# peterrum/dealii-multigrid

Hardware: AMD Instinct MI355X
Metric: DoF/s per V-cycle, 3D octant p=4 (higher is better)
Workload: dtype f64; 1 GPU; 3D octant (GeometryType quadrant) HMG-global p=4 FP64, NRefGlobal=8, SmootherDegree=3, coarse solver direct, f=1, zero Dirichlet (BASELINE.json configs[2]); n_dofs=137199985, n_cells=2127189, n_levels=9, parallelism=1 GPU, chebyshev_start_vector=deal.II's (i mod 11) - mean on the local numbering, fused_transfer_bricks=33509

## Files before the change

### dealii_multigrid_amd/csrc/kernels_apply.hpp

```cpp
#pragma once
#include "kernels_common.hpp"

namespace mgamd
{
#ifdef MGAMD_KERNEL_DEBUG
#define MGAMD_STAMP(k)                         \
  if (args.stamps && tid == 0)                 \
    args.stamps[(size_t)block * 8 + (k)] = wall_clock64();
#define MGAMD_ABLATED(bit) (args.ablate & (bit))
#else
#define MGAMD_STAMP(k)
#define MGAMD_ABLATED(bit) false
#endif

  template <typename T, int P>
  __device__ __forceinline__ void
  interior_diag_terms(const Mats<P, T> &mats, const int t, T &s_K, T &s_M)
  {
    const int tt[3] = {t % P, (t / P) % P, t / (P * P)};
    T         m[3], k[3];
#pragma unroll
    for (int d = 0; d < 3; ++d)
      {
        T dm = T(0), dk = T(0);
        if (tt[d] == 0)
          {
            dm = T(mats.M[P * (P + 1) + P]) + T(mats.M[0]);
            dk = T(mats.K[P * (P + 1) + P]) + T(mats.K[0]);
          }
#pragma unroll
        for (int q = 1; q < P; ++q)
          if (q == tt[d])
            {
              dm = T(mats.M[q * (P + 1) + q]);
              dk = T(mats.K[q * (P + 1) + q]);
            }
        m[d] = dm;
        k[d] = dk;
      }
    s_K = k[0] * m[1] * m[2] + m[0] * k[1] * m[2] + m[0] * m[1] * k[2];
    s_M = m[0] * m[1] * m[2];
  }

  template <typename T, int P, int B, int MODE, bool CONSTR = false, bool WAVE = false, int NTHREADS = 0, bool MASS = true>
// ... 252 lines not shown
        MGAMD_STAMP(4)
      }
#endif
  }

  template <typename T, int P, int B, int MODE_, bool CONSTR, bool MASS>
  __device__ __forceinline__ void
  lattice_apply_persistent_body(const ApplyArgs<T, P> &args, const uint32_t w, const uint32_t stride, unsigned char *smem_raw)
  {
    using G  = Geo<P, B>;
    using IM = InteriorMap<P, B>;
    static_assert(G::SPW == 1 && G::N_INT > 0, "persistent workgroups: one slot per workgroup");
    constexpr int  MODE   = base_mode(MODE_);
    constexpr bool FUSE_R = MODE_ == MODE_RESIDUAL_RESTRICT, FUSE_P = MODE_ == MODE_CHEB_PROLONGATE, FUSE = FUSE_R || FUSE_P;
    static_assert(!FUSE || (!CONSTR && B >= 2 && G::ABLOCK == 256), "fused transfers: plain bricks, 256 threads");
    static_assert(!CONSTR || P == 1, "constrained bricks larger than a family: p = 1 only (LevelTables::build)");
    static_assert(MODE_ != MODE_MASS || !MASS, "the mass pass has no mass TERM: one instantiation, MASS = false");
    constexpr int BC = B >= 2 ? B / 2 : 1, NC = P * BC + 1, NC3 = NC * NC * NC;
    T *bufA = reinterpret_cast<T *>(smem_raw);
    T *bufB = bufA + G::N3;
    T *dtab = bufB + G::N3;

    constexpr int BLOCK = G::ABLOCK;
    constexpr int ITER  = (G::N_INT + BLOCK - 1) / BLOCK;
    constexpr int ITERS = (G::N_SHELL + BLOCK - 1) / BLOCK;
    constexpr int ITC   = FUSE ? (NC3 + BLOCK - 1) / BLOCK : 1;
    constexpr int P3    = P * P * P;
    static_assert(!FUSE || 2 * ITERS <= 15, "two flag bits per shell entry in a 16-bit word");

    const int      tid = threadIdx.x;
    const uint32_t n   = args.g.n_slots;
    if (w >= n)
      return;

    if (is_cheb(MODE))
      {
        for (int t = tid; t < P3; t += BLOCK)
          {
            T sv, s_M;
            interior_diag_terms<T, P>(args.m, t, sv, s_M);
            dtab[t]      = sv;
            dtab[P3 + t] = T(1) / sv;
          }
      }
    constexpr int NI = IM::NI_;
    struct InteriorWalk
    {
      int x, y, z;
      __device__ __forceinline__ int
      pos() const
      {
        return (z * G::N + y) * G::N + x;
      }
      __device__ __forceinline__ int
      type() const
      {
        return (x % P) + P * ((y % P) + P * (z % P));
      }
      __device__ __forceinline__ void
      next()
      {
        constexpr int DZ = BLOCK / (NI * NI), DY = (BLOCK % (NI * NI)) / NI, DX = BLOCK % NI;
        x += DX;
        if (x > NI)
          {
            x -= NI;
            ++y;
          }
        y += DY;
        if (y > NI)
          {
            y -= NI;
            ++z;
          }
        z += DZ;
      }
    };
    const InteriorWalk walk0{tid % NI + 1, (tid / NI) % NI + 1, tid / (NI * NI) + 1};
    auto has_entry = [&](int it) -> bool { return (it + 1) * BLOCK <= G::N_INT || tid + it * BLOCK < G::N_INT; };
    int spos[ITERS];
#pragma unroll
    for (int it = 0; it < ITERS; ++it)
      {
        const int idx = tid + it * BLOCK;
        spos[it]      = idx < G::N_SHELL ? (int)args.g.shell_pos[idx] : -1;
      }
    __syncthreads();

    constexpr bool x_from_b = MODE == MODE_CHEB_FIRST;
    auto load_tables = [&](uint32_t v, uint32_t &slot, uint32_t &base, uint32_t(&sg)[ITERS], double &h, uint32_t &fm, uint32_t &fl,
                           uint32_t(&cg)[ITC]) {
      slot = xcd_contiguous(v, n);
      base = args.g.interior_base[slot];
      h    = args.g.h[slot];
      fm   = 0;
      fl   = 0;
      if constexpr (FUSE)
        {
          fl = args.fused.flags[(size_t)slot * BLOCK + tid];
          const uint32_t *__restrict__ c0 = args.fused.coarse_idx + (size_t)slot * NC3;
#pragma unroll
          for (int it = 0; it < ITC; ++it)
            cg[it] = NT_LOAD(c0 + min(tid + it * BLOCK, NC3 - 1));
        }
      if constexpr (brick_may_be_constrained(B, CONSTR))
        if (args.g.fmask != nullptr)
          fm = args.g.fmask[slot];
      const uint32_t *__restrict__ p0 = args.g.shell_idx + (size_t)slot * G::N_SHELL;
#pragma unroll
      for (int it = 0; it < ITERS; ++it)
        {
          if ((it + 1) * BLOCK <= G::N_SHELL)
            sg[it] = NT_LOAD(p0 + it * BLOCK + tid);
          else
            sg[it] = NT_LOAD(p0 + min(tid + it * BLOCK, G::N_SHELL - 1));
        }
    };
    auto load_values = [&](uint32_t base, const uint32_t(&sg)[ITERS], const uint32_t fl, const uint32_t(&cg)[ITC], T(&xv)[ITER], T(&sv)[ITERS],
                           T(&sbv)[ITERS], T(&cv)[ITC]) {
      const T *__restrict__ in = x_from_b ? args.epi.b : args.src;
#pragma unroll
      for (int it = 0; it < ITER; ++it)
        xv[it] = NT_LOAD(&in[base + (uint32_t)(has_entry(it) ? tid + it * BLOCK : 0)]);
#pragma unroll
      for (int it = 0; it < ITERS; ++it)
        {
          const uint32_t gi = sg[it] < args.gather_limit ? sg[it] : 0;
          sv[it]            = in[gi];
          if (x_from_b)
            sbv[it] = args.epi.dinv[gi];
          if (FUSE_R)
            sbv[it] = args.epi.b[((fl >> (2 * it)) & 1u) ? gi : 0];
        }
      if constexpr (FUSE_P)
        {
#pragma unroll
          for (int it = 0; it < ITC; ++it)
            cv[it] = args.fused.coarse[cg[it] != DEV_INVALID ? cg[it] : 0];
        }
    };

    uint32_t slot, base, sgi[ITERS], fmcur, flcur, cgi[ITC];
    double   hcur;
    T        xg[ITER], sval[ITERS], sb[ITERS], cval[ITC];
    load_tables(w, slot, base, sgi, hcur, fmcur, flcur, cgi);
    load_values(base, sgi, flcur, cgi, xg, sval, sb, cval);

    for (uint32_t v = w;;)
      {
        const uint32_t block    = v;
        (void)block;
        const uint32_t vn       = v + stride;
        const bool     has_next = vn < n;
        MGAMD_STAMP(0)
        const T rh = T(1) / T(hcur);
        if constexpr (MASS && is_cheb(MODE))
          {
            const T c = T(args.sigma) * T(args.g.q[slot]);
            for (int t = tid; t < P3; t += BLOCK)
              {
                T s_K, s_M;
                interior_diag_terms<T, P>(args.m, t, s_K, s_M);
                const T sv   = s_K + c * s_M;
                dtab[t]      = sv;
                dtab[P3 + t] = T(1) / sv;
              }
            if (x_from_b)
              __syncthreads();
          }
        auto interior_dinv = [&](int t) -> T {
          return fabs((double)dtab[t]) > 1.0e-10 * fabs((double)rh) ? rh * dtab[P3 + t] : T(1);
        };
        const bool fused_slot = FUSE && ((__builtin_amdgcn_readfirstlane((int)flcur) >> 15) & 1);
        T          bv[ITER], xo[ITER];
        uint32_t slotn = slot, basen = base, sgn[ITERS], fmn = fmcur, fln = flcur, cgn[ITC];
        double   hn = hcur;
        if (has_next)
          load_tables(vn, slotn, basen, sgn, hn, fmn, fln, cgn);
        {
#pragma unroll
          for (int it = 0; it < ITER; ++it)
            {
              const uint32_t g = base + (uint32_t)(has_entry(it) ? tid + it * BLOCK : 0);
              xo[it]           = T(0);
              bv[it]           = x_from_b ? xg[it] : T(0);
              if (MODE == MODE_CHEB && !FUSE_P && args.epi.xold)
                xo[it] = NT_LOAD(&args.epi.xold[g]);
// ... 53 lines not shown
                    const uint32_t f2 = (flcur >> (2 * it)) & 3u;
                    if (!(f2 & 2u))
                      sval[it] += bufB[spos[it]];
                    if (f2 & 1u)
                      args.fused.scratch[sgi[it]] = sval[it];
                  }
              InteriorWalk wk = walk0;
#pragma unroll
              for (int it = 0; it < ITER; ++it, wk.next())
                if (has_entry(it))
                  {
                    xg[it] += bufB[wk.pos()];
                    NT_STORE(xg[it], &args.fused.x_inout[base + (uint32_t)(tid + it * BLOCK)]);
                  }
            }
        if (x_from_b)
          {
#pragma unroll
            for (int it = 0; it < ITERS; ++it)
              sval[it] = args.epi.c0 * sb[it] * sval[it];
          }
#pragma unroll
        for (int it = 0; it < ITERS; ++it)
          if (spos[it] >= 0)
            bufA[spos[it]] = sgi[it] < args.gather_limit ? sval[it] : T(0);
        {
          InteriorWalk wk = walk0;
#pragma unroll
          for (int it = 0; it < ITER; ++it, wk.next())
            if (has_entry(it))
              bufA[wk.pos()] = x_from_b ? args.epi.c0 * interior_dinv(wk.type()) * bv[it] : xg[it];
        }
        __syncthreads();
        MGAMD_STAMP(1)

        bool any_hanging = false;
        if constexpr (brick_may_be_constrained(B, CONSTR))
          {
            any_hanging = fmcur != 0;
            if (any_hanging)
              brick_constraint_passes<T, P, B, BLOCK>(bufA, args.m, tid, 1, args.g.fmask + slot, false, &fmcur);
          }
        if constexpr (MODE == MODE_MASS)
          mass_sweeps<T, P, B, BLOCK, true, true, false>(bufA, args.m, tid, 1, &hcur, false);
        else
          lattice_sweeps<T, P, B, BLOCK, NoHook, true, (MODE != MODE_CHEB || sizeof(T) == 4), false, MASS>(
            bufA, bufB, args.m, tid, 1, &hcur, NoHook(), false, args.sigma, args.g.q + slot);
        if constexpr (brick_may_be_constrained(B, CONSTR))
          if (any_hanging)
            brick_constraint_passes<T, P, B, BLOCK>(bufA, args.m, tid, 1, args.g.fmask + slot, true, &fmcur);
        MGAMD_STAMP(2)

        T xgn[ITER], svaln[ITERS], sbn[ITERS], cvaln[ITC];
        if (has_next)
          load_values(basen, sgn, fln, cgn, xgn, svaln, sbn, cvaln);

        if (FUSE_R && fused_slot)
          {
            if constexpr (FUSE_R)
              {
                InteriorWalk wk = walk0;
#pragma unroll
                for (int it = 0; it < ITER; ++it, wk.next())
                  if (has_entry(it))
                    bufA[wk.pos()] = bv[it] - bufA[wk.pos()];
#pragma unroll
// ... 52 lines not shown
              if (has_entry(it))
                {
                  const uint32_t g  = base + (uint32_t)(tid + it * BLOCK);
                  const T        ax = bufA[wk.pos()];
                  T              r;
                  if (MODE == MODE_VMULT || MODE == MODE_MASS)
                    r = ax;
                  else if (MODE == MODE_RESIDUAL)
                    r = bv[it] - ax;
                  else
                    {
                      const T dv  = interior_dinv(wk.type());
                      const T xov = MODE == MODE_CHEB_SECOND ? args.epi.c0 * dv * bv[it] : xo[it];
                      const T xv  = x_from_b ? args.epi.c0 * dv * bv[it] : xg[it];
                      if (FUSE_P)
                        r = xv + args.epi.f2 * dv * (bv[it] - ax);
                      else
                        r = xv + args.epi.f1 * (xv - xov) + args.epi.f2 * dv * (bv[it] - ax);
                    }
                  if (MODE == MODE_CHEB && !FUSE_P)
                    store_result(args.epi, g, r);
                  else
                    NT_STORE(r, &args.epi.out[g]);
                }
            MGAMD_STAMP(3)
#pragma unroll
            for (int it = 0; it < ITERS; ++it)
              if (spos[it] >= 0 && sgi[it] < args.scatter_limit)
                atomic_add(&args.tail_acc[sgi[it] - args.n_interior], bufA[spos[it]]);
          }
        MGAMD_STAMP(4)
        if (!has_next)
          break;
        v    = vn;
        slot  = slotn;
        base  = basen;
        hcur  = hn;
        fmcur = fmn;
        flcur = fln;
#pragma unroll
        for (int it = 0; it < ITC; ++it)
          {
            cgi[it]  = cgn[it];
            cval[it] = cvaln[it];
          }
#pragma unroll
        for (int it = 0; it < ITERS; ++it)
          {
            sgi[it]  = sgn[it];
            sval[it] = svaln[it];
            sb[it]   = sbn[it];
          }
#pragma unroll
        for (int it = 0; it < ITER; ++it)
          xg[it] = xgn[it];
        __syncthreads();
      }
  }
#undef MGAMD_STAMP
#undef MGAMD_ABLATED

  constexpr int CELL_WAVES = 4;
  template <typename T, int P>
  constexpr size_t
  cell_wave_lds()
  {
    using G = Geo<P, 1, 64>;
    static_assert(P >= 2, "wave-scoped cells: P >= 2 (at P = 1 the closed-form D^-1 table of lattice_apply_body is per slot, apply_lds_bytes)");
    return (((2 * (size_t)G::SPW * G::N3 + 2 * P * P * P + G::SPW) * sizeof(T) + 15) / 16) * 16;
  }

  constexpr size_t CU_LDS_BYTES = 160 * 1024;
  constexpr int
  wgs_lds_admits(size_t lds_bytes)
  {
    return (int)(CU_LDS_BYTES / lds_bytes);
  }
  constexpr int
  min_of(int a, int b, int c)
  {
    return a < b ? (a < c ? a : c) : (b < c ? b : c);
  }
  template <typename T, int P>
  constexpr size_t
  small_slots_lds_bytes()
  {
    return apply_lds_bytes<T, P, 2>() > CELL_WAVES * cell_wave_lds<T, P>() ? apply_lds_bytes<T, P, 2>() : CELL_WAVES * cell_wave_lds<T, P>();
  }
  template <typename T, int P>
  constexpr int
  brick2_vgpr_cap()
  {
// ... 76 lines not shown
  struct BrickPairArgs
  {
    ApplyArgs<T, P> a;
    SlotGroupDev    g_constrained;
    uint32_t        n_wg_plain;
  };
  static_assert(sizeof(BrickPairArgs<double, MAX_KERNEL_DEGREE>) <= KERNARG_LIMIT, "BrickPairArgs exceeds the kernel-argument segment");
  template <typename T, int P, int B, int MODE>
  __global__ void
  __launch_bounds__((Geo<P, B>::ABLOCK), 1) lattice_apply_pair_kernel(const BrickPairArgs<T, P> args)
  {
    extern __shared__ __align__(16) unsigned char smem_raw[];
    if (blockIdx.x < args.n_wg_plain)
      lattice_apply_body<T, P, B, MODE, false>(args.a, blockIdx.x, args.n_wg_plain, smem_raw);
    else
      {
        ApplyArgs<T, P> a = args.a;
        a.g               = args.g_constrained;
        a.stamps          = nullptr;
        lattice_apply_body<T, P, B, MODE, true>(a, blockIdx.x - args.n_wg_plain, gridDim.x - args.n_wg_plain, smem_raw);
      }
  }

  template <typename T, int P, int B, int MODE, bool MASS>
  __global__ void
  __launch_bounds__((Geo<P, B>::ABLOCK), 2) lattice_apply_persistent_pair_kernel(const BrickPairArgs<T, P> args)
  {
    extern __shared__ __align__(16) unsigned char smem_raw[];
    if (args.n_wg_plain == 0)
      {
        ApplyArgs<T, P> a = args.a;
        a.g               = args.g_constrained;
        a.stamps          = nullptr;
        lattice_apply_persistent_body<T, P, B, base_mode(MODE), true, MASS>(a, blockIdx.x, gridDim.x, smem_raw);
        __syncthreads();
        lattice_apply_persistent_body<T, P, B, MODE, false, MASS>(args.a, blockIdx.x, gridDim.x, smem_raw);
      }
    else if (blockIdx.x < args.n_wg_plain)
      lattice_apply_persistent_body<T, P, B, MODE, false, MASS>(args.a, blockIdx.x, args.n_wg_plain, smem_raw);
    else
      {
        ApplyArgs<T, P> a = args.a;
        a.g               = args.g_constrained;
        a.stamps          = nullptr;
        lattice_apply_persistent_body<T, P, B, base_mode(MODE), true, MASS>(a, blockIdx.x - args.n_wg_plain, gridDim.x - args.n_wg_plain, smem_raw);
      }
  }

  template <typename T, int P>
  struct SmallSlotsArgs
  {
    ApplyArgs<T, P> a;
    SlotGroupDev    g_cells;
    uint32_t        n_wg_bricks;
  };
  static_assert(sizeof(SmallSlotsArgs<double, MAX_KERNEL_DEGREE>) <= KERNARG_LIMIT, "SmallSlotsArgs exceeds the kernel-argument segment");
  template <typename T, int P, int MODE, bool MASS = true>
  __global__ void
  __launch_bounds__(256, (small_slots_wgs_per_cu<T, P>())) lattice_apply_small_kernel(const SmallSlotsArgs<T, P> args)
  {
    extern __shared__ __align__(16) unsigned char smem_raw[];
    if (blockIdx.x < args.n_wg_bricks)
      lattice_apply_body<T, P, 2, MODE, false, false, 256, MASS>(args.a, blockIdx.x, args.n_wg_bricks, smem_raw);
    else
      {
        ApplyArgs<T, P> a = args.a;
        a.g               = args.g_cells;
        a.stamps          = nullptr;
        cell_waves_body<T, P, MODE, MASS>(a, blockIdx.x - args.n_wg_bricks, gridDim.x - args.n_wg_bricks, smem_raw);
      }
  }

  struct CellClusterDev
  {
    const uint32_t *uniq_ptr;
    const uint32_t *uniq_idx;
    const uint16_t *loc;
// ... 683 lines not shown
```

### dealii_multigrid_amd/csrc/kernels_common.hpp

```cpp
#pragma once
#include <hip/hip_runtime.h>
#include <stdint.h>

namespace mgamd
{
  constexpr uint32_t DEV_INVALID = 0xFFFFFFFFu;

  constexpr size_t KERNARG_LIMIT     = 4096;
  constexpr int    MAX_KERNEL_DEGREE = 7;

#ifndef MGAMD_NO_NT_STREAMS
#define NT_LOAD(p) __builtin_nontemporal_load(p)
#define NT_STORE(v, p) __builtin_nontemporal_store(v, p)
#else
#define NT_LOAD(p) (*(p))
#define NT_STORE(v, p) (*(p) = (v))
#endif

  __device__ __forceinline__ uint32_t
  xcd_contiguous(uint32_t b, uint32_t n)
  {
    const uint32_t k = b & 7u, q = n >> 3, r = n & 7u;
    return k * q + (k < r ? k : r) + (b >> 3);
  }

  template <int P, typename S = double>
  struct Mats
  {
    S M[(P + 1) * (P + 1)];
    S K[(P + 1) * (P + 1)];
    S I0[(P + 1) * (P + 1)];
    S I1[(P + 1) * (P + 1)];
    static constexpr int NH = (P + 2) / 2, NO = (P + 1) / 2;
    S                    Me[NH * NH], Mo[NO * NO], Ke[NH * NH], Ko[NO * NO];
  };

  constexpr bool
  brick_may_be_constrained(int B, bool constr)
  {
    return B == 2 || (constr && B > 2);
  }

  template <int P, int B, int THREADS = 256>
  struct Geo
  {
    static constexpr int N       = P * B + 1;
    static constexpr int N3      = N * N * N;
    static constexpr int NI      = N - 2;
    static constexpr int N_INT   = NI > 0 ? NI * NI * NI : 0;
    static constexpr int N_SHELL = N3 - N_INT;
    static constexpr int LINES   = N * N;
    static constexpr int SPW     = LINES >= THREADS ? 1 : THREADS / LINES;
    static constexpr int BLOCK   = ((SPW * LINES + 63) / 64) * 64;
    static constexpr int ABLOCK  = BLOCK > 256 ? 256 : BLOCK;
    static constexpr int ROUNDS  = (SPW * LINES + ABLOCK - 1) / ABLOCK;
  };

// ... 1042 lines not shown
            {
#pragma unroll
              for (int b = 0; b <= P; ++b)
                out[c * P + (mir ? P - b : b)] += T(Eh[ar * (P + 1) + b]) * v;
            }
        }
  }

  template <typename T, int P>
  struct FusedTransferDev
  {
    const uint32_t *flags      = nullptr;
    const uint32_t *coarse_idx = nullptr;
    T               Eh[(P + 1) * (P + 1)];
    T              *coarse  = nullptr;
    T              *x_inout = nullptr;
    T              *scratch = nullptr;
  };

  template <typename T, int P>
  struct ApplyArgs
  {
    SlotGroupDev g;
    Mats<P, T>   m;
    const T     *src;
    T           *tail_acc;
    uint32_t     n_interior;
    unsigned long long *stamps;
    uint32_t     ablate;
    Epilogue<T>  epi;
    uint32_t gather_limit, scatter_limit;
    FusedTransferDev<T, P> fused;
    double sigma = 0.0;
  };
  static_assert(sizeof(ApplyArgs<double, MAX_KERNEL_DEGREE>) <= KERNARG_LIMIT, "ApplyArgs exceeds the kernel-argument segment");

  template <int P, int B, int THREADS = 256>
  struct InteriorMap
  {
    using G                   = Geo<P, B, THREADS>;
    static constexpr int NI_  = G::NI > 0 ? G::NI : 1;
    static constexpr int NIN_ = G::N_INT > 0 ? G::N_INT : 1;
    static constexpr int ITER = (G::SPW * NIN_ + G::ABLOCK - 1) / G::ABLOCK;
    __device__ static __forceinline__ void
    decode(int idx, int nslots, bool &ok, int &sl, int &i, int &lds)
    {
      ok = idx < nslots * NIN_;
      sl = (G::SPW == 1 || !ok) ? 0 : idx / NIN_;
      i  = G::SPW == 1 ? (ok ? idx : 0) : (ok ? idx % NIN_ : 0);
      const int x = i % NI_, y = (i / NI_) % NI_, z = i / (NI_ * NI_);
      lds = sl * G::N3 + ((z + 1) * G::N + (y + 1)) * G::N + x + 1;
    }
  };

}
```

### dealii_multigrid_amd/csrc/level_operator.hpp

```cpp
#pragma once
#include "runtime.hpp"
#include "kernels.hpp"

#include <cmath>
#include <cstring>
#include <map>
#include <mutex>
#include <type_traits>
#include <unordered_map>

namespace mgamd
{
  inline int
  grid_for(size_t n)
  {
    size_t g = (n + 255) / 256;
    if (g > 2048)
      g = 2048;
    if (g < 1)
      g = 1;
    return (int)g;
  }

  template <typename T>
// ... 9 lines not shown
    hipLaunchKernelGGL(vec_dot_final_kernel<>, 1, 256, 0, ctx->stream, ctx->d_partial, g, ctx->d_result);
    HIP_CHECK(hipMemcpyAsync(ctx->h_result, ctx->d_result, sizeof(double), hipMemcpyDeviceToHost, ctx->stream));
    ctx->sync();
    return ctx->h_result[0];
  }

  inline void
  ensure_dynamic_lds(Ctx *ctx, const void *kern, size_t lds)
  {
    static std::mutex                                      m;
    static std::map<std::pair<int, const void *>, size_t> done;
    std::lock_guard<std::mutex>                            lock(m);
    auto                                                   it = done.find({ctx->device, kern});
    if (it != done.end() && it->second >= lds)
      return;
    HIP_CHECK(hipFuncSetAttribute(kern, hipFuncAttributeMaxDynamicSharedMemorySize, (int)lds));
    done[{ctx->device, kern}] = lds;
  }

  template <typename A>
  inline void
  launch_lds(Ctx *ctx, hipStream_t st, void (*kern)(A), int grid, int block, size_t lds, const A &args)
  {
    ensure_dynamic_lds(ctx, reinterpret_cast<const void *>(kern), lds);
    hipLaunchKernelGGL(kern, grid, block, lds, st, args);
  }

  inline int
  resident_workgroups(const Ctx *ctx, int per_cu = 2)
  {
    return std::max(8, per_cu * ctx->n_cu / 8 * 8);
  }

  template <typename A>
  inline void
  launch_persistent(Ctx *ctx, hipStream_t st, void (*kern)(A), int n_work, int per_cu, int block, size_t lds, const A &args)
  {
    launch_lds(ctx, st, kern, std::min(n_work, resident_workgroups(ctx, per_cu)), block, lds, args);
  }

  template <int... Vs, typename F>
  inline bool
  dispatch_value(int v, F &&f)
  {
    return ((v == Vs && (f(std::integral_constant<int, Vs>()), true)) || ...);
  }
  template <typename F>
  inline bool
  dispatch_degree(int p, F &&f)
  {
    return dispatch_value<1, 2, 3, 4, 5, 6, 7>(p, f);
  }
  template <int P, int... Bs, typename F>
  inline bool
  dispatch_brick_size(int B, F &&f)
  {
    return P * B + 1 <= 17 && dispatch_value<Bs...>(B, [&](auto b) {
             if constexpr (P * b() + 1 <= 17)
               f(b);
           });
  }

  template <typename T, int P, int B, int MODE, bool CONSTR = false>
  inline void
  launch_lattice(Ctx *ctx, hipStream_t st, const ApplyArgs<T, P> &a, bool diag)
  {
    using G = Geo<P, B>;
    if (a.g.n_slots == 0)
      return;
    const int grid = (int)((a.g.n_slots + G::SPW - 1) / G::SPW);
    if (diag)
      launch_lds(ctx, st, lattice_diag_kernel<T, P, B, CONSTR>, grid, G::BLOCK, 3 * (size_t)G::SPW * G::N3 * sizeof(T), a);
    else if constexpr (B == 1 && P >= 2)
      {
        using GW = Geo<P, 1, 64>;
        const uint32_t n_w    = (uint32_t)((a.g.n_slots + GW::SPW - 1) / GW::SPW);
        const uint32_t grid_w = (n_w + CELL_WAVES - 1) / CELL_WAVES;
        constexpr size_t lds  = CELL_WAVES * cell_wave_lds<T, P>();
        static_assert(lds <= 64 * 1024, "above the default dynamic-LDS limit the launch has to go through launch_lds");
        hipLaunchKernelGGL((cell_waves_kernel<T, P, MODE>), grid_w, 64 * CELL_WAVES, lds, st, a);
      }
    else if constexpr (persistent_lattice(G::N))
      {
        void (*kern)(ApplyArgs<T, P>) = lattice_apply_persistent_kernel<T, P, B, MODE, CONSTR, false>;
        if constexpr (MODE != MODE_MASS)
          if (a.sigma != 0.0)
            kern = lattice_apply_persistent_kernel<T, P, B, MODE, CONSTR, true>;
        launch_persistent(ctx, st, kern, grid, persistent_wgs_per_cu<T, P>(), G::ABLOCK, apply_lds_bytes<T, P, B>(), a);
      }
    else
      launch_lds(ctx, st, lattice_apply_kernel<T, P, B, MODE, CONSTR>, grid, G::ABLOCK, apply_lds_bytes<T, P, B>(), a);
    HIP_CHECK(hipGetLastError());
  }

  template <typename T>
  struct GroupDev
  {
    int            B = 1, N = 2;
    bool           constrained = false;
    size_t         n_halo      = 0;
    size_t         n_slots = 0;
    DBuf<uint32_t> interior_base, shell_idx;
    DBuf<uint16_t> mask, shell_pos;
    DBuf<double>   h, q, h_cell;
    DBuf<uint32_t> fmask;
    void
    upload_scales(const SlotGroup &g)
    {
      std::vector<double> ah(g.h.size()), ratio(g.h.size());
      bool                any = false;
      for (size_t s = 0; s < g.h.size(); ++s)
        {
          ah[s]    = g.a[s] * g.h[s];
          ratio[s] = g.h[s] * g.h[s] / g.a[s];
          any |= g.a[s] != 1.0;
        }
      h.upload(ah);
      q.upload(ratio);
      if (any)
        h_cell.upload(g.h);
    }
// ... 71 lines not shown
  template <typename T>
  struct FusedTransferHost
  {
    int                 group = -1;
    const uint32_t     *flags = nullptr;
    const uint32_t     *coarse_idx = nullptr;
    uint32_t            nc3 = 0;
    std::vector<double> E;
    const uint8_t      *tail_flags = nullptr;
    const uint32_t     *tail_chunks   = nullptr;
    uint32_t            n_tail_chunks = 0;
    T *coarse = nullptr, *scratch = nullptr, *x_inout = nullptr;
  };
  constexpr bool
  fused_transfer_supported(int p)
  {
    return persistent_brick(p) != 0;
  }

  template <typename T>
  struct LevelOperator : LevelOperatorBase
  {
    int                                       p = 1;
    std::vector<std::unique_ptr<GroupDev<T>>> groups;
    DBuf<T>                                   tail_acc;
    DBuf<uint8_t>                             dinv_code;
    DBuf<T>                                   dinv_table;
    const T                                  *dinv_coded = nullptr;
    int                                       dominant_B = 0;
    uint32_t                                  ablate = 0;
    DBuf<unsigned long long>                  stamps;
    int                                       stamp_mode = -1;
    bool                                      halo_overlap = true;

    struct HaloDev
    {
      DBuf<uint32_t> pack_idx, sh_tail, sh_ptr;
      DBuf<int32_t>  sh_src, sh_owner_src;
      DBuf<T>        send, recv;
    };
    std::unique_ptr<HaloDev> halo;

    struct RobinDev
    {
      DBuf<uint32_t> idx;
      DBuf<uint8_t>  flags;
      DBuf<double>   scale;
      uint32_t       n_faces = 0;
    };
    std::unique_ptr<RobinDev> robin;

    struct DirichletDev
    {
      DBuf<uint32_t> idx;
      DBuf<uint16_t> mask;
      DBuf<double>   scale;
      uint32_t       n_cells = 0;
    };
    std::unique_ptr<DirichletDev> dirichlet;
    struct HangingDev
    {
      DBuf<uint32_t> ptr, col;
      DBuf<double>   val;
      uint32_t       n_rows = 0;
    };
    std::unique_ptr<HangingDev> hanging;

    enum class LaunchKind
    {
      LATTICE,
      LATTICE_CONSTRAINED,
      BRICK_PAIR,
      BRICKS_AND_CELLS,
      BRICKS_AND_CLUSTERS,
      CLUSTERS,
      ROBIN_FACES
    };
    struct LaunchStep
    {
      LaunchKind   kind;
      GroupDev<T> *g, *partner;
      size_t       begin, end;
    };
    struct LaunchPlan
    {
      std::vector<LaunchStep> ordinary, diagonal;
      std::vector<LaunchStep> halo_slots, interior_slots;
    } plan;

    LevelOperator(Ctx *c, const mgamd_dofs *dofs, std::shared_ptr<Comm> cm)
    {
      ctx    = c;
      type   = (int)sizeof(T);
      tables = dofs->tables;
      tria   = dofs->tria;
      p      = tables->p;
      sigma  = tables->sigma;
      if (tables->ls_level && sigma != 0.0)
        throw std::invalid_argument("level operator: mass coefficient " + std::to_string(sigma) +
                                    " on a local-smoothing level: not implemented (refinement-edge matrices have no mass term)");
      if (cm && dofs->halo)
        {
          comm      = cm;
          halo_plan = dofs->halo;
          halo      = std::make_unique<HaloDev>();
          halo->pack_idx.upload(halo_plan->pack_idx);
          halo->sh_tail.upload(halo_plan->sh_tail);
          halo->sh_ptr.upload(halo_plan->sh_ptr);
          halo->sh_src.upload(halo_plan->sh_src);
          halo->sh_owner_src.upload(halo_plan->sh_owner_src);
          halo->send.alloc(std::max<size_t>(halo_plan->pack_idx.size(), 1));
          halo->recv.alloc(std::max<size_t>(halo_plan->pack_idx.size(), 1));
        }
      size_t best = 0;
      for (const SlotGroup &g : tables->groups)
// ... 19 lines not shown
          const size_t work = d->n_slots * (size_t)g.N * g.N * g.N;
          if (work > best)
            {
              best       = work;
              dominant_B = g.B;
            }
          groups.push_back(std::move(d));
        }
      if (const char *e = getenv("MGAMD_ABLATE"))
        ablate = (uint32_t)atoi(e);
      if (const char *e = getenv("MGAMD_STAMP_B"))
        dominant_B = atoi(e);
      halo_overlap = getenv("MGAMD_NO_HALO_OVERLAP") == nullptr;
      if (const char *e = getenv("MGAMD_STAMPS"))
        {
          stamp_mode = atoi(e);
          size_t nwg = 0;
          for (auto &g : groups)
            if (g->B == dominant_B)
              nwg = g->n_slots;
          stamps.alloc(nwg * 8 + 8);
          stamps.zero(ctx->stream);
        }
      tail_acc.alloc(std::max<uint32_t>(tables->n_tail + tables->n_edge, 1));
      tail_acc.zero(ctx->stream);
      if (tables->robin_faces.size())
        {
          robin = std::make_unique<RobinDev>();
          robin->idx.upload(tables->robin_faces.idx);
          robin->flags.upload(tables->robin_faces.flags);
          robin->scale.upload(tables->robin_faces.scale);
          robin->n_faces = (uint32_t)tables->robin_faces.size();
        }
      build_launch_plan();
    }

    void
    build_launch_plan()
    {
      using K        = LaunchKind;
      auto non_empty = [&](int B, bool constrained) -> GroupDev<T> * {
        for (auto &g : groups)
          if (g->n_slots && g->B == B && g->constrained == constrained)
            return g.get();
        return nullptr;
      };
      auto on_its_own = [&](GroupDev<T> *g, size_t begin, size_t end) {
        const K kind = g->has_clusters() ? K::CLUSTERS : (g->constrained ? K::LATTICE_CONSTRAINED : K::LATTICE);
        return LaunchStep{kind, g, nullptr, begin, end};
      };
      for (auto &g : groups)
        if (g->n_slots)
          plan.diagonal.push_back({g->constrained ? K::LATTICE_CONSTRAINED : K::LATTICE, g.get(), nullptr, 0, g->n_slots});

      GroupDev<T> *cells = non_empty(1, false);
      GroupDev<T> *bricks2 = (p >= 2 && cells) ? non_empty(2, false) : nullptr;
      GroupDev<T> *bricks8 = (p == 1 && cells && cells->has_clusters() && dominant_B != 8) ? non_empty(8, false) : nullptr;
      for (auto &gp : groups)
        {
          GroupDev<T> *g = gp.get();
          if (!g->n_slots || (g == cells && (bricks2 || bricks8)))
            continue;
          if (g == bricks2)
            plan.ordinary.push_back({K::BRICKS_AND_CELLS, g, cells, 0, g->n_slots});
          else if (g == bricks8)
            plan.ordinary.push_back({K::BRICKS_AND_CLUSTERS, g, cells, 0, g->n_slots});
          else
// ... 127 lines not shown
      c.n_interior = a.n_interior;
      c.b          = a.epi.b;
      c.dinv       = a.epi.dinv;
      c.c0         = a.epi.c0;
      c.from_b     = first ? 1 : 0;
      c.cluster_offset = 0;
      c.sigma          = a.sigma;
      return c;
    }

    template <int P, bool MASS_ONLY = false>
    void
    launch_clusters(hipStream_t st, const GroupDev<T> &g, const ApplyArgs<T, P> &a, bool first, size_t begin, size_t end)
    {
      ClusterArgs<T> c    = cluster_args(g, a, first, MASS_ONLY);
      c.cluster_offset    = (uint32_t)(begin / CLUSTER_CELLS);
      const uint32_t grid = (uint32_t)((end + CLUSTER_CELLS - 1) / CLUSTER_CELLS) - c.cluster_offset;
      hipLaunchKernelGGL((MASS_ONLY ? cell_cluster_mass_kernel<T> : cell_cluster_apply_kernel<T>), grid, CLUSTER_CELLS, g.cluster_lds_bytes(), st, c);
      HIP_CHECK(hipGetLastError());
    }

    template <int P, int B, int MODE>
    void
    launch_pair(hipStream_t st, const ApplyArgs<T, P> &a, GroupDev<T> *g_constrained)
    {
      using G = Geo<P, B>;
      BrickPairArgs<T, P> pa;
      pa.a             = a;
      pa.g_constrained = g_constrained->view(MODE == MODE_MASS);
      pa.n_wg_plain    = (uint32_t)((a.g.n_slots + G::SPW - 1) / G::SPW);
      const int n_wg   = (int)(pa.n_wg_plain + (uint32_t)((g_constrained->n_slots + G::SPW - 1) / G::SPW));
      if constexpr (persistent_lattice(G::N))
        {
          if (n_wg > resident_workgroups(ctx))
            pa.n_wg_plain = 0;
          void (*kern)(BrickPairArgs<T, P>) = lattice_apply_persistent_pair_kernel<T, P, B, MODE, false>;
          if constexpr (MODE != MODE_MASS)
            if (a.sigma != 0.0)
              kern = lattice_apply_persistent_pair_kernel<T, P, B, MODE, true>;
          launch_persistent(ctx, st, kern, n_wg, 2, G::ABLOCK, apply_lds_bytes<T, P, B>(), pa);
        }
      else if constexpr (MODE != base_mode(MODE))
        throw std::runtime_error("fused transfers need the persistent brick kernel");
      else
        launch_lds(ctx, st, lattice_apply_pair_kernel<T, P, B, MODE>, n_wg, G::ABLOCK, apply_lds_bytes<T, P, B>(), pa);
      HIP_CHECK(hipGetLastError());
    }

    template <int P, int MODE>
    void
    launch_fused(hipStream_t st, ApplyArgs<T, P> &a, size_t begin, GroupDev<T> *partner_constrained, const FusedTransferHost<T> &f)
    {
      if constexpr (fused_transfer_supported(P))
        {
          constexpr int B = persistent_brick(P);
          using G         = Geo<P, B>;
          constexpr int NC = P * B / 2 + 1, NC3 = NC * NC * NC;
          if (f.nc3 != (uint32_t)NC3 || f.E.size() != (size_t)(2 * P + 1) * (P + 1))
            throw std::runtime_error("fused transfer: tables do not match the brick kernel");
          a.fused.flags      = f.flags + begin * G::ABLOCK;
          a.fused.coarse_idx = f.coarse_idx + begin * NC3;
          for (int i = 0; i < (P + 1) * (P + 1); ++i)
            a.fused.Eh[i] = f.E[i];
          for (int ar = 0; ar <= P; ++ar)
            for (int b = 0; b <= P; ++b)
              if (std::fabs(f.E[(2 * P - ar) * (P + 1) + (P - b)] - f.E[ar * (P + 1) + b]) > 1e-14)
                throw std::runtime_error("fused transfer: the 1D embedding is not centro-symmetric");
          a.fused.coarse  = f.coarse;
          a.fused.x_inout = f.x_inout;
          a.fused.scratch = f.scratch;
          if (partner_constrained)
            {
              if constexpr (P == 1)
                return launch_pair<P, B, MODE>(st, a, partner_constrained);
              throw std::runtime_error("brick pair launch: size not instantiated");
            }
          launch_persistent(ctx, st,
                            a.sigma != 0.0 ? lattice_apply_persistent_kernel<T, P, B, MODE, false, true> :
                                             lattice_apply_persistent_kernel<T, P, B, MODE, false, false>,
                            (int)a.g.n_slots, persistent_wgs_per_cu<T, P>(), G::ABLOCK, apply_lds_bytes<T, P, B>(), a);
          HIP_CHECK(hipGetLastError());
        }
      else
        throw std::runtime_error("fused transfers: degree without 17-point lattice kernel");
    }

    template <int MODE>
    void
    launch_bricks_and_clusters(hipStream_t st, const ApplyArgs<T, 1> &a, const GroupDev<T> &gc)
    {
      using G8 = Geo<1, 8>;
      P1SmallArgs<T> sa;
      sa.a           = a;
      sa.c           = cluster_args(gc, a, MODE == MODE_CHEB_FIRST, MODE == MODE_MASS);
      sa.n_wg_bricks = (uint32_t)((a.g.n_slots + G8::SPW - 1) / G8::SPW);
      const uint32_t n_wg_cl = (uint32_t)((gc.n_slots + CLUSTER_CELLS - 1) / CLUSTER_CELLS);
      const size_t   lds     = std::max(apply_lds_bytes<T, 1, 8>(), gc.cluster_lds_bytes());
      hipLaunchKernelGGL((lattice_cluster_kernel<T, MODE>), sa.n_wg_bricks + n_wg_cl, 256, lds, st, sa);
      HIP_CHECK(hipGetLastError());
    }

    template <int P, int MODE>
    void
    launch_bricks_and_cells(hipStream_t st, const ApplyArgs<T, P> &a, const GroupDev<T> &g1)
    {
      using G2 = Geo<P, 2>;
      SmallSlotsArgs<T, P> sa;
      sa.a           = a;
      sa.g_cells     = g1.view(MODE == MODE_MASS);
      sa.n_wg_bricks = (uint32_t)((a.g.n_slots + G2::SPW - 1) / G2::SPW);
      using GW = Geo<P, 1, 64>;
      const uint32_t n_w        = (uint32_t)((g1.n_slots + GW::SPW - 1) / GW::SPW);
      const uint32_t n_wg_cells = (n_w + CELL_WAVES - 1) / CELL_WAVES;
      constexpr size_t lds      = small_slots_lds_bytes<T, P>();
      static_assert(lds <= 64 * 1024, "above the default dynamic-LDS limit the launch has to go through launch_lds");
      hipLaunchKernelGGL((a.sigma == 0.0 || MODE == MODE_MASS ? lattice_apply_small_kernel<T, P, MODE, false> :
                                                                 lattice_apply_small_kernel<T, P, MODE, true>),
                         sa.n_wg_bricks + n_wg_cells, 256, lds, st, sa);
      HIP_CHECK(hipGetLastError());
    }

    template <int P, int MODE_>
    void
    launch_step(hipStream_t st, ApplyArgs<T, P> &a, const LaunchStep &s, bool diag, const FusedTransferHost<T> *fused, bool stamp = false)
    {
      constexpr int MODE = base_mode(MODE_);
      using K            = LaunchKind;
      if (s.kind == K::ROBIN_FACES)
        return launch_robin_faces<P, MODE>(st, a, diag);
      GroupDev<T> *g     = s.g;
      a.g                = g->view(s.begin, s.end, MODE == MODE_MASS);
      a.stamps           = nullptr;
      if constexpr (MODE_ != MODE)
        if (fused && fused->group >= 0 && g == groups[fused->group].get())
          return launch_fused<P, MODE_>(st, a, s.begin, s.partner, *fused);
      if (stamp && stamps.p && s.kind != K::BRICK_PAIR && g->B == dominant_B && !g->constrained && MODE == stamp_mode)
        a.stamps = stamps.p;
      bool done = false;
      switch (s.kind)
        {
          case K::LATTICE:
            if (!dispatch_brick_size<P, 1, 2, 4, 8, 16>(g->B, [&](auto B) { launch_lattice<T, P, B(), MODE>(ctx, st, a, diag); }))
              throw std::runtime_error("unsupported brick size");
            break;
          case K::LATTICE_CONSTRAINED:
            if constexpr (P == 1)
              done = dispatch_brick_size<P, 4, 8, 16>(g->B, [&](auto B) { launch_lattice<T, P, B(), MODE, true>(ctx, st, a, diag); });
            if (!done)
              throw std::runtime_error("constrained bricks of this size/degree are not instantiated");
            break;
          case K::BRICK_PAIR:
            if constexpr (P == 1)
              done = dispatch_brick_size<P, 8, 16>(g->B, [&](auto B) { launch_pair<P, B(), MODE>(st, a, s.partner); });
            if (!done)
              throw std::runtime_error("brick pair launch: size not instantiated");
            break;
          case K::BRICKS_AND_CELLS:
            if constexpr (P >= 2)
              launch_bricks_and_cells<P, MODE>(st, a, *s.partner);
            break;
          case K::BRICKS_AND_CLUSTERS:
            if constexpr (P == 1)
              launch_bricks_and_clusters<MODE>(st, a, *s.partner);
            break;
          case K::CLUSTERS:
            launch_clusters<P, MODE == MODE_MASS>(st, *g, a, MODE == MODE_CHEB_FIRST, s.begin, s.end);
            break;
          case K::ROBIN_FACES:
            break;
        }
    }

    template <int P, int MODE>
    void
    launch_robin_faces(hipStream_t st, const ApplyArgs<T, P> &a, bool diag)
    {
      if constexpr (MODE != MODE_MASS)
        {
          RobinArgs<T, P> r;
          r.idx     = robin->idx.p;
// ... 345 lines not shown
```

Before: 14.95 billion DoF/s.

## Replace static strided persistent scheduling with per-XCD atomic ticket work stealing

Persistent brick kernels now pull their next brick from a per-XCD atomic ticket counter, one counter per launch step, instead of walking a fixed stride. Thread 0 draws a ticket and publishes it through LDS, so the workgroup learns its next slot one iteration ahead. The aim is to even out load imbalance between workgroups with uneven brick costs while keeping slots contiguous within each XCD. It adds an atomic per brick plus an optional environment-variable cap on the persistent grid size. Counters rely on atomicInc wrap-around to reset between launches, which is a correctness risk if a launch does not make exactly the expected number of draws.

```diff
diff --git a/dealii_multigrid_amd/csrc/kernels_apply.hpp b/dealii_multigrid_amd/csrc/kernels_apply.hpp
--- a/dealii_multigrid_amd/csrc/kernels_apply.hpp
+++ b/dealii_multigrid_amd/csrc/kernels_apply.hpp
@@ -8,8 +8,12 @@
   if (args.stamps && tid == 0)                 \
     args.stamps[(size_t)block * 8 + (k)] = wall_clock64();
 #define MGAMD_ABLATED(bit) (args.ablate & (bit))
+#define MGAMD_STAMP_OWNER(w)                   \
+  if (args.stamps && tid == 0)                 \
+    args.stamps[(size_t)block * 8 + 7] = (w) + 1;
 #else
 #define MGAMD_STAMP(k)
+#define MGAMD_STAMP_OWNER(w)
 #define MGAMD_ABLATED(bit) false
 #endif
 
@@ -328,6 +332,11 @@
     const uint32_t n   = args.g.n_slots;
     if (w >= n)
       return;
+    const TicketSchedule sched(args.tickets, w, stride, n);
+    uint32_t *const      ticket_word = reinterpret_cast<uint32_t *>(dtab + 2 * P * P * P);
+    uint32_t             drawn       = 0;
+    if (sched.active && tid == 0)
+      drawn = sched.draw();
 
     if (is_cheb(MODE))
       {
@@ -381,12 +390,14 @@
         const int idx = tid + it * BLOCK;
         spos[it]      = idx < G::N_SHELL ? (int)args.g.shell_pos[idx] : -1;
       }
+    if (sched.active && tid == 0)
+      sched.publish(drawn, ticket_word);
     __syncthreads();
 
     constexpr bool x_from_b = MODE == MODE_CHEB_FIRST;
-    auto load_tables = [&](uint32_t v, uint32_t &slot, uint32_t &base, uint32_t(&sg)[ITERS], double &h, uint32_t &fm, uint32_t &fl,
+    auto load_tables = [&](uint32_t s, uint32_t &slot, uint32_t &base, uint32_t(&sg)[ITERS], double &h, uint32_t &fm, uint32_t &fl,
                            uint32_t(&cg)[ITC]) {
-      slot = xcd_contiguous(v, n);
+      slot = s;
       base = args.g.interior_base[slot];
       h    = args.g.h[slot];
       fm   = 0;
@@ -439,16 +450,19 @@
     uint32_t slot, base, sgi[ITERS], fmcur, flcur, cgi[ITC];
     double   hcur;
     T        xg[ITER], sval[ITERS], sb[ITERS], cval[ITC];
-    load_tables(w, slot, base, sgi, hcur, fmcur, flcur, cgi);
+    load_tables(xcd_contiguous(w, n), slot, base, sgi, hcur, fmcur, flcur, cgi);
     load_values(base, sgi, flcur, cgi, xg, sval, sb, cval);
 
-    for (uint32_t v = w;;)
-      {
-        const uint32_t block    = v;
+    for (;;)
+      {
+        const uint32_t block = slot;
         (void)block;
-        const uint32_t vn       = v + stride;
-        const bool     has_next = vn < n;
+        uint32_t   vn       = slot;
+        const bool has_next = sched.active && sched.take(ticket_word, vn);
+        if (has_next && tid == 0)
+          drawn = sched.draw();
         MGAMD_STAMP(0)
+        MGAMD_STAMP_OWNER(w)
         const T rh = T(1) / T(hcur);
         if constexpr (MASS && is_cheb(MODE))
           {
@@ -568,6 +582,8 @@
               bufA[wk.pos()] = x_from_b ? args.epi.c0 * interior_dinv(wk.type()) * bv[it] : xg[it];
         }
         __syncthreads();
+        if (has_next && tid == 0)
+          sched.publish(drawn, ticket_word);
         MGAMD_STAMP(1)
 
         bool any_hanging = false;
@@ -686,7 +702,6 @@
         MGAMD_STAMP(4)
         if (!has_next)
           break;
-        v    = vn;
         slot  = slotn;
         base  = basen;
         hcur  = hn;
@@ -712,6 +727,7 @@
       }
   }
 #undef MGAMD_STAMP
+#undef MGAMD_STAMP_OWNER
 #undef MGAMD_ABLATED
 
   constexpr int CELL_WAVES = 4;
@@ -854,6 +870,7 @@
         ApplyArgs<T, P> a = args.a;
         a.g               = args.g_constrained;
         a.stamps          = nullptr;
+        a.tickets += 8;
         lattice_apply_persistent_body<T, P, B, base_mode(MODE), true, MASS>(a, blockIdx.x, gridDim.x, smem_raw);
         __syncthreads();
         lattice_apply_persistent_body<T, P, B, MODE, false, MASS>(args.a, blockIdx.x, gridDim.x, smem_raw);
@@ -865,6 +882,7 @@
         ApplyArgs<T, P> a = args.a;
         a.g               = args.g_constrained;
         a.stamps          = nullptr;
+        a.tickets += 8;
         lattice_apply_persistent_body<T, P, B, base_mode(MODE), true, MASS>(a, blockIdx.x - args.n_wg_plain, gridDim.x - args.n_wg_plain, smem_raw);
       }
   }
diff --git a/dealii_multigrid_amd/csrc/kernels_common.hpp b/dealii_multigrid_amd/csrc/kernels_common.hpp
--- a/dealii_multigrid_amd/csrc/kernels_common.hpp
+++ b/dealii_multigrid_amd/csrc/kernels_common.hpp
@@ -23,6 +23,43 @@
     const uint32_t k = b & 7u, q = n >> 3, r = n & 7u;
     return k * q + (k < r ? k : r) + (b >> 3);
   }
+
+  struct TicketSchedule
+  {
+    uint32_t *ctr;
+    uint32_t  first;
+    uint32_t  n_valid;
+    uint32_t  n_draws;
+    bool      active;
+    __device__ __forceinline__
+    TicketSchedule(uint32_t *counters, uint32_t w, uint32_t stride, uint32_t n)
+    {
+      const uint32_t k = w & 7u, q = n >> 3, r = n & 7u;
+      const uint32_t q_k = q + (k < r ? 1u : 0u), W_k = (stride - k + 7u) >> 3;
+      active  = n > stride;
+      ctr     = counters + k;
+      first   = k * q + (k < r ? k : r) + W_k;
+      n_valid = q_k - W_k;
+      n_draws = q_k;
+    }
+    __device__ __forceinline__ uint32_t
+    draw() const
+    {
+      return atomicInc(ctr, n_draws - 1u);
+    }
+    __device__ __forceinline__ void
+    publish(uint32_t t, uint32_t *word) const
+    {
+      *word = t;
+    }
+    __device__ __forceinline__ bool
+    take(const uint32_t *word, uint32_t &item) const
+    {
+      const uint32_t t = (uint32_t)__builtin_amdgcn_readfirstlane((int)*word);
+      item             = first + t;
+      return t < n_valid;
+    }
+  };
 
   template <int P, typename S = double>
   struct Mats
@@ -1131,6 +1168,7 @@
     uint32_t gather_limit, scatter_limit;
     FusedTransferDev<T, P> fused;
     double sigma = 0.0;
+    uint32_t *tickets = nullptr;
   };
   static_assert(sizeof(ApplyArgs<double, MAX_KERNEL_DEGREE>) <= KERNARG_LIMIT, "ApplyArgs exceeds the kernel-argument segment");
 
diff --git a/dealii_multigrid_amd/csrc/level_operator.hpp b/dealii_multigrid_amd/csrc/level_operator.hpp
--- a/dealii_multigrid_amd/csrc/level_operator.hpp
+++ b/dealii_multigrid_amd/csrc/level_operator.hpp
@@ -65,11 +65,17 @@
     return std::max(8, per_cu * ctx->n_cu / 8 * 8);
   }
 
+  inline int
+  persistent_grid(const Ctx *ctx, int n_work, int per_cu, int grid_cap)
+  {
+    const int resident = resident_workgroups(ctx, per_cu);
+    return std::min(n_work, grid_cap > 0 ? std::min(resident, grid_cap) : resident);
+  }
   template <typename A>
   inline void
-  launch_persistent(Ctx *ctx, hipStream_t st, void (*kern)(A), int n_work, int per_cu, int block, size_t lds, const A &args)
-  {
-    launch_lds(ctx, st, kern, std::min(n_work, resident_workgroups(ctx, per_cu)), block, lds, args);
+  launch_persistent(Ctx *ctx, hipStream_t st, void (*kern)(A), int n_work, int per_cu, int block, size_t lds, const A &args, int grid_cap = 0)
+  {
+    launch_lds(ctx, st, kern, persistent_grid(ctx, n_work, per_cu, grid_cap), block, lds, args);
   }
 
   template <int... Vs, typename F>
@@ -96,7 +102,7 @@
 
   template <typename T, int P, int B, int MODE, bool CONSTR = false>
   inline void
-  launch_lattice(Ctx *ctx, hipStream_t st, const ApplyArgs<T, P> &a, bool diag)
+  launch_lattice(Ctx *ctx, hipStream_t st, const ApplyArgs<T, P> &a, bool diag, int grid_cap = 0)
   {
     using G = Geo<P, B>;
     if (a.g.n_slots == 0)
@@ -119,7 +125,7 @@
         if constexpr (MODE != MODE_MASS)
           if (a.sigma != 0.0)
             kern = lattice_apply_persistent_kernel<T, P, B, MODE, CONSTR, true>;
-        launch_persistent(ctx, st, kern, grid, persistent_wgs_per_cu<T, P>(), G::ABLOCK, apply_lds_bytes<T, P, B>(), a);
+        launch_persistent(ctx, st, kern, grid, persistent_wgs_per_cu<T, P>(), G::ABLOCK, apply_lds_bytes<T, P, B>(), a, grid_cap);
       }
     else
       launch_lds(ctx, st, lattice_apply_kernel<T, P, B, MODE, CONSTR>, grid, G::ABLOCK, apply_lds_bytes<T, P, B>(), a);
@@ -257,6 +263,9 @@
     DBuf<unsigned long long>                  stamps;
     int                                       stamp_mode = -1;
     bool                                      halo_overlap = true;
+    static constexpr size_t                   TICKETS_PER_STEP = 16;
+    DBuf<uint32_t>                            ticket_counters;
+    int                                       persistent_grid_cap = 0;
 
     struct HaloDev
     {
@@ -306,6 +315,7 @@
       LaunchKind   kind;
       GroupDev<T> *g, *partner;
       size_t       begin, end;
+      uint32_t    *tickets = nullptr;
     };
     struct LaunchPlan
     {
@@ -391,7 +401,18 @@
           robin->scale.upload(tables->robin_faces.scale);
           robin->n_faces = (uint32_t)tables->robin_faces.size();
         }
+      if (const char *e = getenv("MGAMD_PERSISTENT_GRID"))
+        persistent_grid_cap = std::max(8, atoi(e));
       build_launch_plan();
+      ticket_counters.alloc(TICKETS_PER_STEP * (plan.ordinary.size() + plan.halo_slots.size() + plan.interior_slots.size()));
+      ticket_counters.zero(ctx->stream);
+      uint32_t *next_set = ticket_counters.p;
+      for (std::vector<LaunchStep> *steps : {&plan.ordinary, &plan.halo_slots, &plan.interior_slots})
+        for (LaunchStep &s : *steps)
+          {
+            s.tickets = next_set;
+            next_set += TICKETS_PER_STEP;
+          }
     }
 
     void
@@ -585,13 +606,13 @@
       const int n_wg   = (int)(pa.n_wg_plain + (uint32_t)((g_constrained->n_slots + G::SPW - 1) / G::SPW));
       if constexpr (persistent_lattice(G::N))
         {
-          if (n_wg > resident_workgroups(ctx))
+          if (n_wg > persistent_grid(ctx, n_wg, 2, persistent_grid_cap))
             pa.n_wg_plain = 0;
           void (*kern)(BrickPairArgs<T, P>) = lattice_apply_persistent_pair_kernel<T, P, B, MODE, false>;
           if constexpr (MODE != MODE_MASS)
             if (a.sigma != 0.0)
               kern = lattice_apply_persistent_pair_kernel<T, P, B, MODE, true>;
-          launch_persistent(ctx, st, kern, n_wg, 2, G::ABLOCK, apply_lds_bytes<T, P, B>(), pa);
+          launch_persistent(ctx, st, kern, n_wg, 2, G::ABLOCK, apply_lds_bytes<T, P, B>(), pa, persistent_grid_cap);
         }
       else if constexpr (MODE != base_mode(MODE))
         throw std::runtime_error("fused transfers need the persistent brick kernel");
@@ -631,7 +652,7 @@
           launch_persistent(ctx, st,
                             a.sigma != 0.0 ? lattice_apply_persistent_kernel<T, P, B, MODE, false, true> :
                                              lattice_apply_persistent_kernel<T, P, B, MODE, false, false>,
-                            (int)a.g.n_slots, persistent_wgs_per_cu<T, P>(), G::ABLOCK, apply_lds_bytes<T, P, B>(), a);
+                            (int)a.g.n_slots, persistent_wgs_per_cu<T, P>(), G::ABLOCK, apply_lds_bytes<T, P, B>(), a, persistent_grid_cap);
           HIP_CHECK(hipGetLastError());
         }
       else
@@ -684,6 +705,7 @@
       GroupDev<T> *g     = s.g;
       a.g                = g->view(s.begin, s.end, MODE == MODE_MASS);
       a.stamps           = nullptr;
+      a.tickets          = s.tickets;
       if constexpr (MODE_ != MODE)
         if (fused && fused->group >= 0 && g == groups[fused->group].get())
           return launch_fused<P, MODE_>(st, a, s.begin, s.partner, *fused);
@@ -693,12 +715,12 @@
       switch (s.kind)
         {
           case K::LATTICE:
-            if (!dispatch_brick_size<P, 1, 2, 4, 8, 16>(g->B, [&](auto B) { launch_lattice<T, P, B(), MODE>(ctx, st, a, diag); }))
+            if (!dispatch_brick_size<P, 1, 2, 4, 8, 16>(g->B, [&](auto B) { launch_lattice<T, P, B(), MODE>(ctx, st, a, diag, persistent_grid_cap); }))
               throw std::runtime_error("unsupported brick size");
             break;
           case K::LATTICE_CONSTRAINED:
             if constexpr (P == 1)
-              done = dispatch_brick_size<P, 4, 8, 16>(g->B, [&](auto B) { launch_lattice<T, P, B(), MODE, true>(ctx, st, a, diag); });
+              done = dispatch_brick_size<P, 4, 8, 16>(g->B, [&](auto B) { launch_lattice<T, P, B(), MODE, true>(ctx, st, a, diag, persistent_grid_cap); });
             if (!done)
               throw std::runtime_error("constrained bricks of this size/degree are not instantiated");
             break;
```

Result: faster. 15.69 billion DoF/s (median of 6 runs) (+4.9%).
